# xingbpshen/nested-diffusion

Hardware: AMD Instinct MI355X
Metric: denoising-steps*images/sec (K=5,T=100,224^2) (higher is better)
Workload: dtype f32

## Files before the change

include/nested_diffusion.h:

```cpp
#ifndef NESTED_DIFFUSION_H
#define NESTED_DIFFUSION_H

#include <stddef.h>
#include <stdint.h>

#ifdef __cplusplus
extern "C" {
#endif

#define ND_OK 0
#define ND_ERR_ARG (-1)
#define ND_ERR_HIP (-2)
#define ND_ERR_STATE (-3)

#define ND_ACT_NONE 0
#define ND_ACT_SOFTPLUS 1
#define ND_ACT_RELU 2
#define ND_ACT_GELU 3

typedef struct nd_handle_s *nd_handle;

typedef struct {
    int32_t y_dim;
    int32_t data_dim;
// ... 21 lines not shown
    const float *lin2_w, *lin2_b, *emb2;
    const float *un2_w, *un2_b, *un2_mean, *un2_var;
    const float *lin3_w, *lin3_b, *emb3;
    const float *un3_w, *un3_b, *un3_mean, *un3_var;
    const float *lin4_w, *lin4_b;
} nd_member_weights;

const char *nd_last_error(void);
const char *nd_version(void);

int nd_create(const nd_config *cfg, nd_handle *out);
int nd_destroy(nd_handle h);
size_t nd_workspace_bytes(const nd_config *cfg);
int nd_bind_workspace(nd_handle h, void *workspace_dev, size_t bytes);

int nd_load_member(nd_handle h, int member, const nd_member_weights *w, void *stream);

int nd_set_schedule(nd_handle h, const float *alphas_dev, const float *omabs_dev, int T, void *stream);

int nd_encode(nd_handle h, int member0, int n_members, const float *x_dev, int B, void *stream);

int nd_eps_theta(nd_handle h, int member, const float *y_dev, const float *yhat_dev, int t,
                 float *eps_out_dev, int B, int mc, void *stream);

int nd_p_sample(nd_handle h, int member, const float *y_dev, const float *yhat_dev, const float *ymean_dev,
                const float *z_dev, int t, float *y_out_dev, int B, int mc, void *stream);

int nd_sample(nd_handle h, int member0, int n_members, const float *yhat_dev, const float *ymean_dev,
              const float *noise_dev, float *y0_out_dev, float *seq_out_dev, int B, int mc, int T,
              int use_graph, void *stream);

int nd_set_profiling(nd_handle h, int enable);
long long nd_resident_weight_bytes(nd_handle h, int block);
int nd_profile_read(nd_handle h, float *out_us, int *n_samples);
int nd_profile_probe_nodes(nd_handle h);

int nd_set_input_flag(nd_handle h, uint32_t *flag_host_visible);

int nd_set_loop_form(nd_handle h, int mode, float skew_us);
int nd_loop_form(nd_handle h);
int nd_persist_status(nd_handle h, int reset);

int nd_member_buffer(nd_handle h, int member, int which, float *dst_dev, int rows, void *stream);

size_t nd_packed_bytes(int R, int K, int dtype);
int nd_pack_rows(const float *src_dev, void *dst_packed_dev, int R, int K, int dtype, void *stream);

size_t nd_linear_workspace_bytes(int M, int K, int N, int dtype);
int nd_linear(const float *x_dev, const void *w_packed_dev, const float *scale_dev, const float *shift_dev,
              float *out_dev, int M, int K, int N, int act, int dtype, void *workspace_dev, size_t workspace_bytes,
              void *stream);

int nd_skinny_plan(int K, int N, int M, int n_members, int dtype, int mode, int *out6);
int nd_skinny_row_fragments(int M);

int nd_step_plan(int feature_dim, int M, int n_members, int dtype, int *out8);

size_t nd_gemm_workspace_bytes(int M, int K, int N, int dtype);
int nd_gemm_bias_act(const float *x_dev, const void *w_dev, const float *bias_dev, const float *residual_dev,
                     float *out_dev, int M, int K, int N, int act, int dtype, void *workspace_dev, size_t workspace_bytes,
                     void *stream);

size_t nd_split_bytes(int rows, int K);
int nd_split_rows(const float *x_dev, void *out_split_dev, int rows, int K, void *stream);
int nd_join_rows(const void *in_split_dev, float *x_dev, int rows, int K, void *stream);
size_t nd_gemm_split_workspace_bytes(int M, int K, int N);
// ... 168 lines not shown
```

nested_diffusion_amd/_lib.py:

```python
from __future__ import annotations

import ctypes as C
import os
from typing import Optional

HERE = os.path.dirname(os.path.abspath(__file__))
LIB_PATH = os.environ.get("ND_LIB_PATH") or os.path.join(HERE, "libnd_hip.so")

ND_ACT_NONE, ND_ACT_SOFTPLUS, ND_ACT_RELU, ND_ACT_GELU = 0, 1, 2, 3
ND_DTYPE_F32, ND_DTYPE_F16 = 0, 1
ND_DTYPE_F32_SPLIT = 2


def dtype_code(dtype) -> int:
    name = str(dtype).replace("torch.", "").lower()
    if name in ("f32", "fp32", "float32", "0"):
        return ND_DTYPE_F32
    if name in ("f16", "fp16", "float16", "half", "1"):
        return ND_DTYPE_F16
    raise ValueError(f"operand dtype must be 'f32' or 'f16', got {dtype!r}")

MEMBER_WEIGHT_FIELDS = [
    ("enc0_w", "encoder_x.0.weight"), ("enc0_b", "encoder_x.0.bias"),
    ("bn0_w", "encoder_x.1.weight"), ("bn0_b", "encoder_x.1.bias"),
    ("bn0_mean", "encoder_x.1.running_mean"), ("bn0_var", "encoder_x.1.running_var"),
    ("enc3_w", "encoder_x.3.weight"), ("enc3_b", "encoder_x.3.bias"),
    ("bn1_w", "encoder_x.4.weight"), ("bn1_b", "encoder_x.4.bias"),
    ("bn1_mean", "encoder_x.4.running_mean"), ("bn1_var", "encoder_x.4.running_var"),
    ("enc6_w", "encoder_x.6.weight"), ("enc6_b", "encoder_x.6.bias"),
    ("norm_w", "norm.weight"), ("norm_b", "norm.bias"),
    ("norm_mean", "norm.running_mean"), ("norm_var", "norm.running_var"),
    ("lin1_w", "lin1.lin.weight"), ("lin1_b", "lin1.lin.bias"), ("emb1", "lin1.embed.weight"),
    ("un1_w", "unetnorm1.weight"), ("un1_b", "unetnorm1.bias"),
    ("un1_mean", "unetnorm1.running_mean"), ("un1_var", "unetnorm1.running_var"),
    ("lin2_w", "lin2.lin.weight"), ("lin2_b", "lin2.lin.bias"), ("emb2", "lin2.embed.weight"),
    ("un2_w", "unetnorm2.weight"), ("un2_b", "unetnorm2.bias"),
    ("un2_mean", "unetnorm2.running_mean"), ("un2_var", "unetnorm2.running_var"),
    ("lin3_w", "lin3.lin.weight"), ("lin3_b", "lin3.lin.bias"), ("emb3", "lin3.embed.weight"),
    ("un3_w", "unetnorm3.weight"), ("un3_b", "unetnorm3.bias"),
    ("un3_mean", "unetnorm3.running_mean"), ("un3_var", "unetnorm3.running_var"),
    ("lin4_w", "lin4.weight"), ("lin4_b", "lin4.bias"),
]

# ... 30 lines not shown
    _fields_ = [("w_packed", C.c_void_p * 4), ("bias", C.c_void_p * 4)]


class NdAdamStep(C.Structure):
    _fields_ = [(n, C.c_float) for n in ("beta1", "one_minus_beta1", "beta2", "one_minus_beta2", "step_size", "sqrt_bc2", "eps")]


class NdBatchOut(C.Structure):
    _fields_ = [(n, C.c_void_p) for n in ("samples", "prob", "vote", "probs", "yhat")]


_vp, _i, _sz, _f = C.c_void_p, C.c_int, C.c_size_t, C.c_float
SIGNATURES = {
    "nd_last_error": (C.c_char_p, []),
    "nd_version": (C.c_char_p, []),
    "nd_create": (_i, [C.POINTER(NdConfig), C.POINTER(_vp)]),
    "nd_destroy": (_i, [_vp]),
    "nd_workspace_bytes": (_sz, [C.POINTER(NdConfig)]),
    "nd_bind_workspace": (_i, [_vp, _vp, _sz]),
    "nd_load_member": (_i, [_vp, _i, C.POINTER(NdMemberWeights), _vp]),
    "nd_set_schedule": (_i, [_vp, _vp, _vp, _i, _vp]),
    "nd_encode": (_i, [_vp, _i, _i, _vp, _i, _vp]),
    "nd_eps_theta": (_i, [_vp, _i, _vp, _vp, _i, _vp, _i, _i, _vp]),
    "nd_p_sample": (_i, [_vp, _i, _vp, _vp, _vp, _vp, _i, _vp, _i, _i, _vp]),
    "nd_sample": (_i, [_vp, _i, _i, _vp, _vp, _vp, _vp, _vp, _i, _i, _i, _i, _vp]),
    "nd_set_profiling": (_i, [_vp, _i]),
    "nd_set_input_flag": (_i, [_vp, _vp]),
    "nd_set_loop_form": (_i, [_vp, _i, C.c_float]),
    "nd_loop_form": (_i, [_vp]),
    "nd_persist_status": (_i, [_vp, _i]),
    "nd_profile_read": (_i, [_vp, C.POINTER(C.c_float), C.POINTER(_i)]),
    "nd_profile_probe_nodes": (_i, [_vp]),
    "nd_resident_weight_bytes": (C.c_longlong, [_vp, _i]),
    "nd_member_buffer": (_i, [_vp, _i, _i, _vp, _i, _vp]),
    "nd_seed": (_i, [_vp, C.c_uint64, C.c_uint32]),
    "nd_philox_normal": (_i, [_vp, _i, _i, _i, _i, _i, C.c_uint64, C.c_uint32, C.c_uint32, _vp]),
    "nd_philox_raw": (_i, [_vp, _vp, _i, C.c_uint32, C.c_uint32, _vp]),
    "nd_cond_workspace_bytes": (_sz, [C.POINTER(NdCondConfig)]),
    "nd_cond_create": (_i, [C.POINTER(NdCondConfig), C.POINTER(_vp)]),
    "nd_cond_destroy": (_i, [_vp]),
    "nd_cond_get_config": (C.POINTER(NdCondConfig), [_vp]),
    "nd_cond_bind_workspace": (_i, [_vp, _vp, _sz]),
    "nd_cond_set_patch_embed": (_i, [_vp, C.POINTER(NdPatchEmbedWeights)]),
    "nd_cond_set_block": (_i, [_vp, _i, C.POINTER(NdVitBlockWeights)]),
    "nd_cond_set_mlp": (_i, [_vp, _i, C.POINTER(NdMlpWeights)]),
    "nd_vit_block": (_i, [_vp, _i, _vp, _vp, _i, _i, _vp]),
    "nd_guiding_prediction": (_i, [_vp, _vp, _vp, _vp, _i, _vp]),
    "nd_predict_batch": (_i, [_vp, _vp, _vp, _vp, C.POINTER(NdBatchOut), _i, _i, _i, _f, _i, _vp]),
    "nd_packed_bytes": (_sz, [_i, _i, _i]),
    "nd_pack_rows": (_i, [_vp, _vp, _i, _i, _i, _vp]),
    "nd_linear_workspace_bytes": (_sz, [_i, _i, _i, _i]),
    "nd_linear": (_i, [_vp, _vp, _vp, _vp, _vp, _i, _i, _i, _i, _i, _vp, _sz, _vp]),
    "nd_skinny_plan": (_i, [_i, _i, _i, _i, _i, _i, C.POINTER(_i)]),
    "nd_step_plan": (_i, [_i, _i, _i, _i, C.POINTER(_i)]),
    "nd_skinny_row_fragments": (_i, [_i]),
    "nd_gemm_workspace_bytes": (_sz, [_i, _i, _i, _i]),
    "nd_gemm_bias_act": (_i, [_vp, _vp, _vp, _vp, _vp, _i, _i, _i, _i, _i, _vp, _sz, _vp]),
    "nd_split_bytes": (_sz, [_i, _i]),
    "nd_split_rows": (_i, [_vp, _vp, _i, _i, _vp]),
    "nd_join_rows": (_i, [_vp, _vp, _i, _i, _vp]),
    "nd_gemm_split_workspace_bytes": (_sz, [_i, _i, _i]),
    "nd_gemm_split": (_i, [_vp, _vp, _vp, _vp, _vp, _vp, _i, _i, _i, _i, _vp, _sz, _vp]),
    "nd_layernorm": (_i, [_vp, _vp, _vp, _vp, _i, _i, _f, _vp]),
    "nd_layernorm_split": (_i, [_vp, _vp, _vp, _vp, _i, _i, _f, _vp]),
    "nd_attention": (_i, [_vp, _vp, _i, _i, _i, _i, _i, _vp]),
    "nd_attention_split": (_i, [_vp, _vp, _i, _i, _i, _i, _vp]),
# ... 93 lines not shown
```

nested_diffusion_amd/csrc/nd_common.hpp:

```cpp
#pragma once
#include <type_traits>
#include <mutex>
#include <unordered_map>
#include <hip/hip_runtime.h>
#include <stdint.h>

typedef float f32x4 __attribute__((ext_vector_type(4)));
typedef _Float16 f16x8 __attribute__((ext_vector_type(8)));
typedef _Float16 f16x4 __attribute__((ext_vector_type(4)));

#define ND_ACT_NONE 0
#define ND_ACT_SOFTPLUS 1
#define ND_ACT_RELU 2
#define ND_ACT_GELU 3

__device__ __forceinline__ float nd_softplus(float x) {
#pragma clang fp contract(off)
    const float u = expf(-fabsf(x));
    const float w = 1.0f + u;
    const float c = (w - 1.0f) - u;
    const float r = fmaxf(x, 0.0f) + __builtin_fmaf(-c, __builtin_amdgcn_rcpf(w), logf(w));
    return x > 20.0f ? x : r;
}

// ... 140 lines not shown
}

typedef __attribute__((address_space(1))) const f32x4 nd_gf4;
template <bool NT>
__device__ __forceinline__ float4 nd_ld16(const float* p) {
    const nd_gf4* g = (const nd_gf4*)p;
    const f32x4 v = NT ? __builtin_nontemporal_load(g) : *g;
    return make_float4(v[0], v[1], v[2], v[3]);
}

#ifdef ND_WG_TIMING
__device__ long long* nd_dbg_times = nullptr;
#endif

__device__ __forceinline__ float nd_ldg(const float* p) {
    return *(const __attribute__((address_space(1))) float*)p;
}

#ifndef ND_PF_TWO
#define ND_PF_TWO 0
#endif
#ifndef ND_PF_LEAD
#define ND_PF_LEAD 0
#endif
struct SkinnyDesc {
    const float* x;
    const float* w;
    const float* scale;
    const float* shift;
    float* out;
    const float* pw;
    float* part;
    int K, N, C, act, out_packed;
    int keep;
    const float* pf;
};

#define ND_INLINE_DESCS 8
struct SkinnyInline { SkinnyDesc d[ND_INLINE_DESCS]; };

template <typename T>
__device__ __forceinline__ T nd_ldc(const __attribute__((address_space(4))) void* p) {
    static_assert(sizeof(T) % 4 == 0, "word-sized structs only");
    T out;
    const __attribute__((address_space(4))) uint32_t* w = (const __attribute__((address_space(4))) uint32_t*)p;
    uint32_t* o = reinterpret_cast<uint32_t*>(&out);
#pragma unroll
    for (unsigned i = 0; i < sizeof(T) / 4; ++i) o[i] = w[i];
    return out;
}

#define ND_SKINNY_STATIC_LDS (60 * 1024)
__host__ __device__ constexpr int nd_skinny_red_bytes(int waves, int nf, int mt) { return waves * nf * mt * 1024; }
template <int MT, int NF, int WAVES, int U, int MODE, bool NT, int H = 0>
__global__ __launch_bounds__(WAVES * 64) void k_skinny(SkinnyInline di, const SkinnyDesc* __restrict__ table, int nm,
                                                       int M, int t, int cps) {
    const int tid = threadIdx.x, lane = tid & 63;
#ifdef ND_WG_TIMING
    const long long dbg_t0 = wall_clock64();
#endif
    const int wave = __builtin_amdgcn_readfirstlane(tid >> 6);
    typedef const __attribute__((address_space(4))) char* nd_cbytes;
    const nd_cbytes dsrc = table ? (nd_cbytes)(uintptr_t)table : (nd_cbytes)__builtin_amdgcn_kernarg_segment_ptr();
    const int K = nd_ldc<SkinnyDesc>(dsrc).K, N = nd_ldc<SkinnyDesc>(dsrc).N;
    const int nch = H ? K >> 5 : K >> 4, nfr = (N + 15) >> 4, mtiles = (M + 15) >> 4;
    const int wpm = gridDim.x / nm;
    const int g = blockIdx.x / wpm, j = blockIdx.x - g * wpm;
    const int base = nfr / wpm, rem = nfr - base * wpm;
    const int nact = base + (j < rem ? 1 : 0);
// ... 80 lines not shown
                                const float wv = jj == 0 ? w[u][f].x : jj == 1 ? w[u][f].y : jj == 2 ? w[u][f].z : w[u][f].w;
                                const float xv = jj == 0 ? x[u][mt].x : jj == 1 ? x[u][mt].y : jj == 2 ? x[u][mt].z : x[u][mt].w;
                                acc[f][mt] = __builtin_amdgcn_mfma_f32_16x16x4f32(wv, xv, acc[f][mt], 0, 0, 0);
                            }
                        }
        };
        auto G = [&](int i) { return min(wave + i * WAVES, glast); };
        int i = 0;
        if (ngw > 0) LD(wA, xA, G(0));
        constexpr int NL = U * (NFA + MT), NM = U * (H ? 1 : 4) * NFA * MT, MR = NM / NL > 0 ? NM / NL : 1;
#define ND_MIX()                                                                                     \
        _Pragma("unroll") for (int q_ = 0; q_ < NL; ++q_) {                                          \
            __builtin_amdgcn_sched_group_barrier(0x020, 1, 0);                                       \
            __builtin_amdgcn_sched_group_barrier(0x008, MR, 0);                                      \
        }                                                                                            \
        __builtin_amdgcn_sched_barrier(0);
        const int pf_at = ngw > ND_PF_LEAD ? (ngw - ND_PF_LEAD) & ~1 : 0;
        for (; i + 1 < ngw; i += 2) {
            if (MODE != 2 && pfp[0] && i == pf_at && ND_PF_LEAD > 0) {
                pfv += nd_ldg(pfp[0]) + nd_ldg(pfp[1]);
                if (ND_PF_TWO) pfv += nd_ldg(pfp[0] + (size_t)WAVES * U * 256) + nd_ldg(pfp[1] + (size_t)WAVES * U * 256);
            }
            LD(wB, xB, G(i + 1));
            MMA(wA, xA);
            ND_MIX()
            LD(wA, xA, G(i + 2));
            MMA(wB, xB);
            ND_MIX()
        }
#undef ND_MIX
        if (ND_PF_LEAD == 0 && MODE != 2 && pfp[0]) pfv += nd_ldg(pfp[0]) + nd_ldg(pfp[1]);
        if (i < ngw) MMA(wA, xA);
    };
    const bool nt_here = NT && !d.keep;
    if (nact == NF) {
        if (nt_here) run(std::true_type{}, std::true_type{});
        else run(std::false_type{}, std::true_type{});
    } else {
        if (nt_here) run(std::true_type{}, std::false_type{});
        else run(std::false_type{}, std::false_type{});
    }
    for (int c = ngroups * U + wave; c < nck; c += WAVES) {
#pragma unroll
        for (int f = 0; f < NF; ++f) {
            const float4 w4 = nd_ld16<false>(wp[f] + (size_t)c * 256 + lane4);
            const float wv[4] = {w4.x, w4.y, w4.z, w4.w};
#pragma unroll
            for (int mt = 0; mt < MT; ++mt) {
                const float4 x4 = nd_ld16<false>(xp[mt] + (size_t)c * 256 + lane4);
                const float xv[4] = {x4.x, x4.y, x4.z, x4.w};
                if (H) acc[f][mt] = __builtin_amdgcn_mfma_f32_16x16x32_f16(nd_as_h8(w4), nd_as_h8(x4), acc[f][mt], 0, 0, 0);
                else {
#pragma unroll
                    for (int jj = 0; jj < 4; ++jj) acc[f][mt] = __builtin_amdgcn_mfma_f32_16x16x4f32(wv[jj], xv[jj], acc[f][mt], 0, 0, 0);
                }
            }
        }
    }
#ifdef ND_WG_TIMING
    const long long dbg_t1 = wall_clock64();
#endif
    if (ND_PF_LEAD < 0 && MODE != 2 && pfp[0]) {
        pfv += nd_ldg(pfp[0]) + nd_ldg(pfp[1]);
        if (ND_PF_TWO) pfv += nd_ldg(pfp[0] + (size_t)WAVES * U * 256) + nd_ldg(pfp[1] + (size_t)WAVES * U * 256);
    }
    if (MODE != 2) {
        if (tid < NF * 16) { ssc[tid >> 4][tid & 15] = r_sc; ssh[tid >> 4][tid & 15] = r_sh; }
// ... 337 lines not shown
```

nested_diffusion_amd/csrc/nd_persist.hip:

```cpp
#include "nd_persist.hpp"
#include <cstddef>

typedef unsigned u32x4 __attribute__((ext_vector_type(4)));
typedef __attribute__((address_space(1))) unsigned* nd_gu32;

#ifdef ND_PERSIST_TIMING
__device__ long long* nd_persist_times = nullptr;
extern "C" int nd_debug_set_persist_times(void* dev_ptr) {
    return hipMemcpyToSymbol(HIP_SYMBOL(nd_persist_times), &dev_ptr, sizeof(void*)) == hipSuccess ? 0 : -1;
}
#define PS_STAMP(k) do { const long long now_ = wall_clock64(); ps_acc[k] += now_ - ps_last; ps_last = now_; } while (0)
#else
#define PS_STAMP(k) do { } while (0)
#endif

#define PS_WAVES 4
#define PS_MT 2
#define PS_U 2

__device__ __forceinline__ unsigned ps_ld_sc1(const unsigned* p) { return __hip_atomic_load((nd_gu32)p, __ATOMIC_RELAXED, __HIP_MEMORY_SCOPE_AGENT); }
__device__ __forceinline__ void ps_st_sc1(unsigned* p, unsigned v) { __hip_atomic_store((nd_gu32)p, v, __ATOMIC_RELAXED, __HIP_MEMORY_SCOPE_AGENT); }
__device__ __forceinline__ float ps_ldf_sc1(const float* p) {
    return __hip_atomic_load((__attribute__((address_space(1))) float*)p, __ATOMIC_RELAXED, __HIP_MEMORY_SCOPE_AGENT);
}
// ... 93 lines not shown
#ifdef ND_PERSIST_TIMING
    long long ps_acc[9] = {0, 0, 0, 0, 0, 0, 0, 0, 0}, ps_last = 0;
#endif

    {
        const SkinnyDesc d3 = PS_ARG_G(ka, SkinnyDesc, l3, g);
        const StepIO io = PS_ARG(ka, StepIO, io);
        for (int e = tid; e < NF * C * 16; e += WAVES * 64) {
            const int f = e / (C * 16), c = (e / 16) % C, nl = e & 15;
            const int n = min(fi0 + f, nfr - 1) * 16 + nl;
            smem[L::pws + e] = (f < nact) ? nd_ldg(d3.pw + (size_t)c * F + n) : 0.f;
        }
        for (int p = tid; p < pairs; p += WAVES * 64) {
            const int m = p / C, c = p - m * C, b = m % B;
            smem[L::syh + p] = nd_ldg(io.yhat + g * io.yhat_ms + (size_t)b * C + c);
            smem[L::sym + p] = nd_ldg(io.ymean + g * io.ymean_ms + (size_t)b * C + c);
        }
    }
    __syncthreads();

    const int ngroups = nch / U;
    const int ngw = ngroups > wave ? (ngroups - wave + WAVES - 1) / WAVES : 0;
    const int glast = ngroups > 0 ? ngroups - 1 : 0;
    float (*const red)[NF * MT * 256] = reinterpret_cast<float (*)[NF * MT * 256]>(smem + L::red);

    auto poison = [&]() {
        if (j != 0) return;
        const StepIO io = PS_ARG(ka, StepIO, io);
        for (int p = tid; p < pairs; p += WAVES * 64) ND_GW(io.y0_out)[g * io.y0_ms + p] = __builtin_nanf("");
    };

    auto layer = [&](auto modec, int t) -> bool {
        constexpr int MODE = decltype(modec)::value;
        const float* wbase; const float* xbase; float* obase; int keep;
        float r_sc = 1.0f, r_sh = 0.0f;
        {
            const SkinnyDesc d = MODE == 0 ? PS_ARG_G(ka, SkinnyDesc, l2, g) : PS_ARG_G(ka, SkinnyDesc, l3, g);
            wbase = d.w; xbase = d.x; obase = MODE == 0 ? d.out : d.part; keep = d.keep;
            if (tid < NF * 16) {
                const int n = min(min(fi0 + (tid >> 4), nfr - 1) * 16 + (tid & 15), F - 1);
                r_sc = nd_ldg(d.scale + (size_t)t * F + n);
                r_sh = nd_ldg(d.shift + (size_t)t * F + n);
            }
        }
        const __amdgpu_buffer_rsrc_t rx = ps_rsrc(xbase);
        const float* wp[NF];
#pragma unroll
        for (int f = 0; f < NF; ++f) wp[f] = wbase + (size_t)min(fi0 + f, nfr - 1) * nch * 256;
        f32x4 acc[NF][MT];
#pragma unroll
        for (int f = 0; f < NF; ++f)
#pragma unroll
            for (int mt = 0; mt < MT; ++mt) acc[f][mt] = f32x4{0.f, 0.f, 0.f, 0.f};
        bool alive = true;
        auto run = [&](auto ntc, auto fullc) {
            constexpr bool NTV = decltype(ntc)::value, FULL = decltype(fullc)::value;
            constexpr int NFA = FULL ? NF : (NF > 1 ? NF - 1 : 1);
            float4 wA[U][NFA], xA[U][MT], wB[U][NFA], xB[U][MT];
            auto LDW = [&](float4 (&w)[U][NFA], int grp) {
                const size_t go = (size_t)grp * U * 256;
#pragma unroll
                for (int u = 0; u < U; ++u)
#pragma unroll
                    for (int f = 0; f < NFA; ++f) w[u][f] = nd_ld16<NTV>(wp[f] + go + u * 256 + lane4);
            };
            auto LDX = [&](float4 (&x)[U][MT], int grp) {
#pragma unroll
                for (int u = 0; u < U; ++u)
#pragma unroll
                    for (int mt = 0; mt < MT; ++mt)
                        x[u][mt] = ps_ld16_sc1(rx, lane * 16, ((min(mt, mtiles - 1) * nch + grp * U + u) * 1024));
// ... 300 lines not shown
```

nested_diffusion_amd/csrc/nd_sampler.hip:

```cpp
#include "nd_common.hpp"
#include "nd_step.hpp"
#include "nd_cond_gemm.hpp"
#include "nd_b9.hpp"
#include "nd_persist.hpp"
#include "nd_rng.hpp"
#include "../../include/nested_diffusion.h"

#include <map>
#include <string>
#include <tuple>
#include <vector>
#include <cstdio>
#include <cstdarg>
#include <cstring>
#include <cstdlib>

static thread_local std::string g_err;
extern "C" const char* nd_last_error(void) { return g_err.c_str(); }
#ifdef ND_WG_TIMING
int nd_debug_set_wg_times_m0(void*); int nd_debug_set_wg_times_m1(void*); int nd_debug_set_wg_times_m2(void*);
extern "C" int nd_debug_set_wg_times(void* dev_ptr) {
    return (nd_debug_set_wg_times_m0(dev_ptr) | nd_debug_set_wg_times_m1(dev_ptr) | nd_debug_set_wg_times_m2(dev_ptr)) ? -1 : 0;
}
#endif
// ... 289 lines not shown
        case 1: return (void*)k_step_final<1>;
        case 2: return (void*)k_step_final<2>;
        case 3: return (void*)k_step_final<3>;
        case 4: return (void*)k_step_final<4>;
        case 5: return (void*)k_step_final<5>;
        case 6: return (void*)k_step_final<6>;
        case 7: return (void*)k_step_final<7>;
        default: return (void*)k_step_final<8>;
    }
}

__global__ void k_fold_bn(float* scale, float* shift, const float* lin_b, const float* bn_w, const float* bn_b,
                          const float* bn_mean, const float* bn_var, int N) {
    const int n = blockIdx.x * blockDim.x + threadIdx.x;
    if (n >= N) return;
    const double s = (double)bn_w[n] / sqrt((double)bn_var[n] + 1e-5);
    const double o = (double)bn_b[n] - (double)bn_mean[n] * s;
    scale[n] = (float)s;
    shift[n] = (float)(s * (double)lin_b[n] + o);
}
__global__ void k_fold_steps(float* A, float* Cc, const float* emb, const float* lin_b, const float* bn_w, const float* bn_b,
                             const float* bn_mean, const float* bn_var, int T, int N) {
    const size_t i = (size_t)blockIdx.x * blockDim.x + threadIdx.x;
    if (i >= (size_t)T * N) return;
    const int n = (int)(i % N);
    const double s = (double)bn_w[n] / sqrt((double)bn_var[n] + 1e-5);
    const double o = (double)bn_b[n] - (double)bn_mean[n] * s;
    const double g = (double)emb[i];
    A[i] = (float)(s * g);
    Cc[i] = (float)(s * g * (double)lin_b[n] + o);
}

#define ND_KEEP_BYTES 208.0e6
enum { L_ENC0 = 0, L_ENC1 = 1, L_ENC2 = 2, L_LIN2 = 3, L_LIN3 = 4, L_LIN2S = 5, L_LIN3S = 6, L_COUNT = 7 };

struct MemberHost {
    bool loaded = false;
    float *sc0, *sh0, *sc1, *sh1, *sc2, *sh2;
    float *A[3], *Cc[3];
    float *w_enc0, *w_enc3, *w_enc6, *w_lin2, *w_lin3;
    float *w_lin1, *w_lin4, *b_lin4;
    float *e0, *e1, *xe, *ybuf, *h1, *h2, *epart, *splitk;
    void *w_lin2s = nullptr, *w_lin3s = nullptr, *h1s = nullptr, *h2s = nullptr;
    bool h_split = false;
};

struct GraphKey {
    int m0, nm, B, mc, T;
    const void *yhat, *ymean, *noise, *y0, *seq;
    bool operator<(const GraphKey& o) const {
        return std::tie(m0, nm, B, mc, T, yhat, ymean, noise, y0, seq) <
               std::tie(o.m0, o.nm, o.B, o.mc, o.T, o.yhat, o.ymean, o.noise, o.y0, o.seq);
    }
};

int nd_guiding_prediction_first(nd_cond c, const float* images, float* logits_out, float* yhat_out, int B, int n_used, void* stream);
unsigned long long nd_cond_serial(nd_cond c);

struct BatchKey {
    unsigned long long cond;
    const void *images, *noise, *samples, *prob, *vote, *probs, *yhat;
    int B, mc, T;
    unsigned temp_bits;
    bool profiling;
    bool operator<(const BatchKey& o) const {
        return std::tie(cond, images, noise, samples, prob, vote, probs, yhat, B, mc, T, temp_bits, profiling) <
               std::tie(o.cond, o.images, o.noise, o.samples, o.prob, o.vote, o.probs, o.yhat, o.B, o.mc, o.T, o.temp_bits, o.profiling);
    }
};

struct nd_handle_s {
    nd_config cfg{};
    char* ws = nullptr;
    size_t ws_bytes = 0;
    std::vector<MemberHost> members;
    MemberDev* members_dev = nullptr;
    SkinnyDesc* descs_dev = nullptr;
    std::vector<SkinnyDesc> descs_host;
    std::vector<MemberDev> members_host;
    SkinnyDesc* spk_dev = nullptr;
    SplitKEpiDesc* spke_dev = nullptr;
    float *alphas = nullptr, *omabs = nullptr;
    float* xpack = nullptr;
    float* tile_ws = nullptr;
    bool b9 = false;
    unsigned long long* rng_state = nullptr;
    unsigned* input_seq = nullptr;
    unsigned* input_flag = nullptr;
    unsigned* persist_bar = nullptr;
    int persist_mode = 0;
    int persist_skew_ticks = 0;
    bool persist_last = false;
    float* noise_ws = nullptr;
    float* logits_ws = nullptr;
    int sched_T = 0;
    int NT = 0, S0 = 0;
    bool enc_splitk = false;
    int half = 0;
    std::map<GraphKey, hipGraphExec_t> graphs;
    std::map<BatchKey, hipGraphExec_t> batch_graphs;
    hipStream_t capture_stream = nullptr;
    int encoded_B = -1;
    bool profiling = false;
    std::vector<hipEvent_t> probe_events;
    int probe_steps = 0;
    int probe_nodes = 0;
};

static inline size_t al256(size_t x) { return (x + 255) & ~(size_t)255; }

struct Carver {
    char* base; size_t off = 0;
    template <typename T> T* take(size_t count) {
        T* p = base ? reinterpret_cast<T*>(base + off) : nullptr;
        off = al256(off + count * sizeof(T));
        return p;
    }
};

static void carve(nd_handle_s* h, char* base, size_t* total) {
    const nd_config& c = h->cfg;
    const size_t K = c.n_members, H = c.hidden_dim, F = c.feature_dim, T = c.n_steps, C = c.y_dim, D = c.data_dim;
    const size_t mB = c.max_batch, mM = c.max_rows;
    const size_t pB = ((mB + 15) / 16) * 16, pM = ((mM + 15) / 16) * 16;
    h->NT = (int)((F + 15) / 16);
    h->half = c.operand_dtype == ND_DTYPE_F16;
    const size_t wdiv = h->half ? 2 : 1;
    h->enc_splitk = nd_use_splitk(c.data_dim);
    h->S0 = h->enc_splitk ? nd_skinny_launch<2>(c.data_dim, c.hidden_dim, c.max_batch, 1, h->half).S : 0;
    Carver cv{base};
    h->members_dev = cv.take<MemberDev>(K);
// ... 103 lines not shown
    HIP_CHECK(hipMemset(h->rng_state, 0, 2 * sizeof(unsigned long long)));
    HIP_CHECK(hipMemset(h->persist_bar, 0, ND_PERSIST_BAR_WORDS * sizeof(unsigned)));
    HIP_CHECK(hipMemset(h->input_seq, 0, sizeof(unsigned)));
    return ND_OK;
}

extern "C" int nd_seed(nd_handle h, uint64_t seed, uint32_t first_image) {
    if (!h || !h->ws) return nd_set_err(ND_ERR_STATE, "workspace not bound");
    const unsigned long long st[2] = {(unsigned long long)seed, (unsigned long long)first_image << 32};
    HIP_CHECK(hipDeviceSynchronize());
    HIP_CHECK(hipMemcpy(h->rng_state, st, sizeof st, hipMemcpyHostToDevice));
    return ND_OK;
}

extern "C" int nd_set_schedule(nd_handle h, const float* alphas_dev, const float* omabs_dev, int T, void* stream) {
    if (!h || !h->ws) return nd_set_err(ND_ERR_STATE, "workspace not bound");
    if (!alphas_dev || !omabs_dev) return nd_set_err(ND_ERR_ARG, "NULL schedule");
    if (T < 1 || T > h->cfg.n_steps) return nd_set_err(ND_ERR_ARG, "T=%d outside [1,%d]", T, h->cfg.n_steps);
    hipStream_t st = (hipStream_t)stream;
    HIP_CHECK(hipMemcpyAsync(h->alphas, alphas_dev, sizeof(float) * T, hipMemcpyDeviceToDevice, st));
    HIP_CHECK(hipMemcpyAsync(h->omabs, omabs_dev, sizeof(float) * T, hipMemcpyDeviceToDevice, st));
    h->sched_T = T;
    return ND_OK;
}

static void launch_pack(const float* src, float* dst, int R, int K, int half, hipStream_t st) {
    const size_t n4 = (size_t)((R + 15) / 16) * 16 * K / (half ? 8 : 4);
    const size_t want = (n4 + 255) / 256;
    const dim3 grid((unsigned)(want > 8192 ? 8192 : want));
    if (half) hipLaunchKernelGGL(k_pack_rows_h, grid, dim3(256), 0, st, src, reinterpret_cast<_Float16*>(dst), R, K);
    else hipLaunchKernelGGL(k_pack_rows, grid, dim3(256), 0, st, src, dst, R, K);
}

extern "C" int nd_load_member(nd_handle h, int k, const nd_member_weights* w, void* stream) {
    if (!h || !h->ws) return nd_set_err(ND_ERR_STATE, "workspace not bound");
    if (k < 0 || k >= h->cfg.n_members) return nd_set_err(ND_ERR_ARG, "member %d out of range", k);
    if (!w) return nd_set_err(ND_ERR_ARG, "weights is NULL");
    const void* const* pp = reinterpret_cast<const void* const*>(w);
    for (size_t i = 0; i < sizeof(nd_member_weights) / sizeof(void*); ++i)
        if (!pp[i]) return nd_set_err(ND_ERR_ARG, "nd_member_weights pointer #%zu is NULL", i);
    hipStream_t st = (hipStream_t)stream;
    const nd_config& c = h->cfg;
    const int H = c.hidden_dim, F = c.feature_dim, T = c.n_steps, C = c.y_dim, D = c.data_dim;
    MemberHost& m = h->members[k];
    auto g1 = [](int n) { return dim3((n + 255) / 256); };
    hipLaunchKernelGGL(k_fold_bn, g1(H), dim3(256), 0, st, m.sc0, m.sh0, w->enc0_b, w->bn0_w, w->bn0_b, w->bn0_mean, w->bn0_var, H);
    hipLaunchKernelGGL(k_fold_bn, g1(H), dim3(256), 0, st, m.sc1, m.sh1, w->enc3_b, w->bn1_w, w->bn1_b, w->bn1_mean, w->bn1_var, H);
    hipLaunchKernelGGL(k_fold_bn, g1(F), dim3(256), 0, st, m.sc2, m.sh2, w->enc6_b, w->norm_w, w->norm_b, w->norm_mean, w->norm_var, F);
    const float* embs[3] = {w->emb1, w->emb2, w->emb3};
    const float* lb[3] = {w->lin1_b, w->lin2_b, w->lin3_b};
    const float* bw[3] = {w->un1_w, w->un2_w, w->un3_w};
    const float* bb[3] = {w->un1_b, w->un2_b, w->un3_b};
    const float* bm[3] = {w->un1_mean, w->un2_mean, w->un3_mean};
    const float* bv[3] = {w->un1_var, w->un2_var, w->un3_var};
    const size_t tot = (size_t)T * F;
    for (int l = 0; l < 3; ++l)
        hipLaunchKernelGGL(k_fold_steps, dim3((unsigned)((tot + 255) / 256)), dim3(256), 0, st, m.A[l], m.Cc[l], embs[l], lb[l],
                           bw[l], bb[l], bm[l], bv[l], T, F);
    launch_pack(w->enc0_w, m.w_enc0, H, D, h->half, st);
    launch_pack(w->enc3_w, m.w_enc3, H, H, h->half, st);
    launch_pack(w->enc6_w, m.w_enc6, F, H, h->half, st);
    launch_pack(w->lin2_w, m.w_lin2, F, F, h->half, st);
    launch_pack(w->lin3_w, m.w_lin3, F, F, h->half, st);
    if (h->b9) {
        int rc = nd_split_rows(w->lin2_w, m.w_lin2s, F, F, st);
        if (rc == ND_OK) rc = nd_split_rows(w->lin3_w, m.w_lin3s, F, F, st);
        if (rc != ND_OK) return rc;
        HIP_CHECK(nd_cond_gemm_b9_prepare());
    }
    HIP_CHECK(hipMemcpyAsync(m.w_lin1, w->lin1_w, sizeof(float) * F * 2 * C, hipMemcpyDeviceToDevice, st));
    HIP_CHECK(hipMemcpyAsync(m.w_lin4, w->lin4_w, sizeof(float) * C * F, hipMemcpyDeviceToDevice, st));
    HIP_CHECK(hipMemcpyAsync(m.b_lin4, w->lin4_b, sizeof(float) * C, hipMemcpyDeviceToDevice, st));
    HIP_CHECK(hipGetLastError());

    MemberDev md{m.w_lin1, m.b_lin4, m.A[0], m.Cc[0], m.xe, m.h1, m.ybuf, m.epart, h->half};
    const int opk = h->half ? 2 : 1;
    SkinnyDesc ds[L_COUNT];
    ds[L_ENC0] = SkinnyDesc{h->xpack, m.w_enc0, m.sc0, m.sh0, m.e0, nullptr, nullptr, D, H, C, ND_ACT_SOFTPLUS, opk};
    ds[L_ENC1] = SkinnyDesc{m.e0, m.w_enc3, m.sc1, m.sh1, m.e1, nullptr, nullptr, H, H, C, ND_ACT_SOFTPLUS, opk};
    ds[L_ENC2] = SkinnyDesc{m.e1, m.w_enc6, m.sc2, m.sh2, m.xe, nullptr, nullptr, H, F, C, ND_ACT_NONE, 1};
    ds[L_LIN2] = SkinnyDesc{m.h1, m.w_lin2, m.A[1], m.Cc[1], m.h2, nullptr, nullptr, F, F, C, ND_ACT_SOFTPLUS, opk};
    ds[L_LIN3] = SkinnyDesc{m.h2, m.w_lin3, m.A[2], m.Cc[2], nullptr, m.w_lin4, m.epart, F, F, C, ND_ACT_SOFTPLUS, 0};
    if (!getenv("ND_NO_XPREFETCH")) { ds[L_LIN2].pf = m.w_lin3; ds[L_LIN3].pf = m.w_lin2; }
    ds[L_LIN2S] = ds[L_LIN2]; ds[L_LIN3S] = ds[L_LIN3];
    if (h->b9) {
        ds[L_LIN2S].x = (const float*)m.h1s; ds[L_LIN2S].w = (const float*)m.w_lin2s; ds[L_LIN2S].out = (float*)m.h2s; ds[L_LIN2S].out_packed = 3;
        ds[L_LIN3S].x = (const float*)m.h2s; ds[L_LIN3S].w = (const float*)m.w_lin3s;
    }
    {
        const double mat = (double)F * F * (h->half ? 2.0 : 4.0);
        const char* keep_mb = getenv("ND_KEEP_MB");
        const int n_keep = (int)((keep_mb ? atof(keep_mb) * 1e6 : ND_KEEP_BYTES) / mat);
        ds[L_LIN2].keep = k < n_keep;
        ds[L_LIN3].keep = c.n_members + k < n_keep;
        if (const char* plan = getenv("ND_KEEP_PLAN")) {
            int a = 0, b = 0;
            if (sscanf(plan, "%d,%d", &a, &b) == 2) { ds[L_LIN2].keep = k < a; ds[L_LIN3].keep = k < b; }
        }
    }
    HIP_CHECK(hipStreamSynchronize(st));
    HIP_CHECK(hipMemcpy(h->members_dev + k, &md, sizeof md, hipMemcpyHostToDevice));
    h->members_host.resize(c.n_members);
    h->descs_host.resize((size_t)L_COUNT * c.n_members);
    h->members_host[k] = md;
    for (int l = 0; l < L_COUNT; ++l) {
        h->descs_host[(size_t)l * c.n_members + k] = ds[l];
        HIP_CHECK(hipMemcpy(h->descs_dev + (size_t)l * c.n_members + k, &ds[l], sizeof(SkinnyDesc), hipMemcpyHostToDevice));
    }
    if (h->enc_splitk) {
        SkinnyDesc sd{h->xpack, m.w_enc0, nullptr, nullptr, nullptr, nullptr, m.splitk, D, H, C, ND_ACT_NONE, 0};
        SplitKEpiDesc se{m.splitk, m.sc0, m.sh0, m.e0, H, 0 , ND_ACT_SOFTPLUS, opk};
        HIP_CHECK(hipMemcpy(h->spk_dev + k, &sd, sizeof sd, hipMemcpyHostToDevice));
        HIP_CHECK(hipMemcpy(h->spke_dev + k, &se, sizeof se, hipMemcpyHostToDevice));
    }
    m.loaded = true;
    drop_graphs(h);
    return ND_OK;
}

static int check_range(nd_handle_s* h, int m0, int nm) {
    if (!h || !h->ws) return nd_set_err(ND_ERR_STATE, "workspace not bound");
    if (m0 < 0 || nm < 1 || m0 + nm > h->cfg.n_members) return nd_set_err(ND_ERR_ARG, "member range [%d,%d) invalid", m0, m0 + nm);
    for (int k = m0; k < m0 + nm; ++k)
        if (!h->members[k].loaded) return nd_set_err(ND_ERR_STATE, "member %d not loaded", k);
    return ND_OK;
}

template <int MODE>
static hipError_t launch_skinny(const SkinnyDesc* table, int K, int N, int M, int t, int nm, int half, hipStream_t st) {
    return nd_launch_skinny(nd_skinny_launch<MODE>(K, N, M, nm, half), SkinnyDesc{}, table, nm, M, t, st);
}
// ... 56 lines not shown
    HIP_CHECK(launch_skinny<0>(h->descs_dev + (size_t)L_ENC1 * K + m0, H, H, B, 0, nm, h->half, st));
    HIP_CHECK(launch_skinny<0>(h->descs_dev + (size_t)L_ENC2 * K + m0, H, F, B, 0, nm, h->half, st));
    HIP_CHECK(hipGetLastError());
    h->encoded_B = B;
    return ND_OK;
}

extern "C" int nd_member_buffer(nd_handle h, int k, int which, float* dst_dev, int rows, void* stream) {
    if (!h || !dst_dev) return nd_set_err(ND_ERR_ARG, "bad argument");
    if (k < 0 || k >= h->cfg.n_members) return nd_set_err(ND_ERR_ARG, "member out of range");
    if (which < 0 || which > 4) return nd_set_err(ND_ERR_ARG, "which=%d unknown", which);
    if (rows < 1 || rows > h->cfg.max_rows) return nd_set_err(ND_ERR_ARG, "rows out of range");
    const bool enc = which == 0 || which >= 3;
    if (enc && rows > h->cfg.max_batch) return nd_set_err(ND_ERR_ARG, "%s holds at most max_batch rows", which == 0 ? "xe" : which == 3 ? "e0" : "e1");
    if (!h->ws) return nd_set_err(ND_ERR_STATE, "workspace not bound");
    MemberHost& m = h->members[k];
    const float* src = which == 0 ? m.xe : which == 1 ? m.h1 : which == 2 ? m.h2 : which == 3 ? m.e0 : m.e1;
    const int W = which >= 3 ? h->cfg.hidden_dim : h->cfg.feature_dim;
    if (!enc && m.h_split) return nd_join_rows(which == 1 ? m.h1s : m.h2s, dst_dev, rows, W, stream);
    const size_t n4 = (size_t)((rows + 15) / 16) * 16 * W / 4;
    if (h->half && which != 0)
        hipLaunchKernelGGL(k_unpack_rows_h, dim3((unsigned)((n4 / 2 + 255) / 256)), dim3(256), 0, (hipStream_t)stream,
                           reinterpret_cast<const _Float16*>(src), dst_dev, rows, W);
    else
        hipLaunchKernelGGL(k_unpack_rows, dim3((unsigned)((n4 + 255) / 256)), dim3(256), 0, (hipStream_t)stream, src, dst_dev, rows, W);
    HIP_CHECK(hipGetLastError());
    return ND_OK;
}

extern "C" long long nd_resident_weight_bytes(nd_handle h, int block) {
    if (!h || block < 0 || block > 1 || h->descs_host.empty()) return -1;
    const int K = h->cfg.n_members, F = h->cfg.feature_dim;
    long long n = 0;
    for (int k = 0; k < K; ++k)
        if (h->members[k].loaded && h->descs_host[(size_t)(block ? L_LIN3 : L_LIN2) * K + k].keep) n += (long long)F * F * (h->half ? 2 : 4);
    return n;
}

extern "C" int nd_set_profiling(nd_handle h, int enable) {
    if (!h) return nd_set_err(ND_ERR_ARG, "handle is NULL");
    if (h->profiling != (enable != 0)) drop_graphs(h);
    h->profiling = enable != 0;
    return ND_OK;
}

extern "C" int nd_set_loop_form(nd_handle h, int mode, float skew_us) {
    if (!h) return nd_set_err(ND_ERR_ARG, "handle is NULL");
    if (mode != 0 && mode != 1) return nd_set_err(ND_ERR_ARG, "mode must be 0 (per-step kernels) or 1 (one launch per loop)");
    if (skew_us > 1e6f) return nd_set_err(ND_ERR_ARG, "skew_us out of range");
    h->persist_mode = mode;
    if (skew_us >= 0.f) h->persist_skew_ticks = (int)(skew_us * 100.0f);
    drop_graphs(h);
    return ND_OK;
}

extern "C" int nd_loop_form(nd_handle h) { return h && h->persist_last ? 1 : 0; }

extern "C" int nd_persist_status(nd_handle h, int reset) {
    if (!h || !h->ws) return nd_set_err(ND_ERR_STATE, "workspace not bound");
    HIP_CHECK(hipDeviceSynchronize());
    unsigned flag = 0;
    HIP_CHECK(hipMemcpy(&flag, h->persist_bar + ND_PERSIST_ERR_WORD, sizeof flag, hipMemcpyDeviceToHost));
    if (reset && flag) HIP_CHECK(hipMemset(h->persist_bar, 0, ND_PERSIST_BAR_WORDS * sizeof(unsigned)));
    return flag ? 1 : 0;
}

static int count_event_record_nodes(hipGraph_t g) {
    size_t n = 0;
    if (hipGraphGetNodes(g, nullptr, &n) != hipSuccess) return -1;
// ... 407 lines not shown
```

nested_diffusion_amd/engine.py:

```python
from __future__ import annotations

import ctypes as C
import os
from typing import Dict, Optional, Sequence, Tuple

import torch

from . import _lib
from ._lib import MEMBER_WEIGHT_FIELDS, NdBatchOut, NdConfig, NdMemberWeights, check, ptr


def _require_gpu(device) -> torch.device:
    device = torch.device(device)
    if device.type != "cuda" or not torch.cuda.is_available():
        raise _lib.NdError("nested_diffusion_amd needs an MI355X (torch device 'cuda'); there is no CPU fallback")
    return device


class EnsembleEngine:

    def __init__(self, y_dim: int, data_dim: int, hidden_dim: int, feature_dim: int, n_steps: int,
                 n_members: int = 1, max_batch: int = 32, max_rows: Optional[int] = None, device="cuda", dtype="f32"):
        self.device = _require_gpu(device)
        self.lib = _lib.load()
# ... 101 lines not shown
        check(self.lib.nd_set_loop_form(self.h, 1 if one_launch else 0, float(skew_us)), "nd_set_loop_form")

    def loop_form(self) -> str:
        return "one_launch" if self.lib.nd_loop_form(self.h) else "graph_nodes"

    def persist_status(self, reset: bool = False) -> bool:
        rc = self.lib.nd_persist_status(self.h, 1 if reset else 0)
        if rc < 0:
            check(rc, "nd_persist_status")
        if rc != 0:
            raise _lib.NdError("one-launch sampling loop: a barrier wait was abandoned (the grid was not resident at once -- another "
                               "process on this device?); results of that call are invalid.  ND_PERSIST=0 selects the per-step form")
        return True

    def set_profiling(self, enable: bool) -> None:
        check(self.lib.nd_set_profiling(self.h, 1 if enable else 0), "nd_set_profiling")

    def profile_read(self):
        torch.cuda.current_stream(self.device).synchronize()
        us = (C.c_float * 4)()
        n = C.c_int(0)
        check(self.lib.nd_profile_read(self.h, us, C.byref(n)), "nd_profile_read")
        self.probe_overhead_us = float(us[3])
        return float(us[0]), float(us[1]), float(us[3]), int(n.value)

    def probe_nodes(self) -> int:
        return int(self.lib.nd_profile_probe_nodes(self.h))

    def resident_weight_bytes(self) -> Tuple[int, int]:
        a, b = self.lib.nd_resident_weight_bytes(self.h, 0), self.lib.nd_resident_weight_bytes(self.h, 1)
        if a < 0 or b < 0:
            raise _lib.NdError("nd_resident_weight_bytes: members not loaded")
        return int(a), int(b)

    def step_plan(self, M: int, n_members: Optional[int] = None) -> Dict[str, object]:
        out = (C.c_int * 8)()
        n_members = self.K if n_members is None else n_members
        check(self.lib.nd_step_plan(self.F, int(M), int(n_members), self.dtype, out), "nd_step_plan")
        tile = bool(out[0])
        b9 = tile and self.dtype == _lib.ND_DTYPE_F32 and self.F % 32 == 0 and n_members <= 8 and not os.environ.get("ND_STEP_F32_MFMA")
        name = (("k_cond_gemm_b9<{0,1}> (LDS-tiled 128x128 ConditionalLinear blocks on the bf16 matrix pipe, nine exact bf16 pair products "
                 "per fp32 product, K members per launch)" if b9 else
                 "k_cond_gemm<{0,1}> (LDS-tiled 128x128 f32-MFMA ConditionalLinear blocks, K members per launch)") if tile else
                "k_skinny<MT,NF,4,U,{0,1}> (weight-streaming lin2 / lin3+lin4 ConditionalLinear blocks, K members per launch)")
        plan = {"kernel": "k_cond_gemm" if tile else "k_skinny", "b9": bool(b9), "name": name, "workgroups": out[1], "whole_tiles": out[2],
                "remainder_tiles": out[3], "split": out[4], "partials": out[5], "TM": out[6], "TN": out[7]}
        if not tile:
            o6 = (C.c_int * 6)()
            check(self.lib.nd_skinny_plan(self.F, self.F, int(M), int(n_members), self.dtype, 1, o6), "nd_skinny_plan")
            mt = self.lib.nd_skinny_row_fragments(int(M))
            if mt < 1:
                check(mt, "nd_skinny_row_fragments")
            plan["stream"] = {"grid": (o6[0], o6[1], o6[2]), "NF": o6[3], "MT": mt, "chunks_per_slab": o6[4], "threads": o6[5]}
        return plan

    def static_buffers(self, n_members: int, B: int, mc: int, T: int, seq: bool) -> Dict[str, torch.Tensor]:
        key = (n_members, B, mc, T, seq)
        buf = self._static.get(key)
        if buf is None:
            M, C_ = B * mc, self.C
            dev = self.device
            buf = {"yhat": torch.empty(n_members, B, C_, device=dev), "ymean": torch.empty(n_members, B, C_, device=dev),
                   "noise": torch.empty(n_members, T, M, C_, device=dev), "y0": torch.empty(n_members, M, C_, device=dev)}
            if seq:
                buf["seq"] = torch.empty(n_members, T + 1, M, C_, device=dev)
            self._static[key] = buf
# ... 84 lines not shown
```

Baseline: 790,500.

## Make cache residency of skinny-layer weights a per-fragment range plan

Replaces the per-member boolean 'keep' flag (which decided whether a whole FxF weight matrix is loaded with temporal hints or non-temporal loads) with a per-workgroup fragment range [keep_lo, keep_hi). A planner fills these ranges under a byte budget using several layouts: whole matrices, matrices plus a fractional one, or a heavy-first slice spread evenly across members. New API calls let the residency be set at runtime. The f32 default keeps the matrix layout with the same budget, so f32 behaviour should be close to the old whole-matrix policy. f16 defaults to a heavy+even layout with a slightly smaller budget. The kernel now checks the range per workgroup, which adds a small amount of per-workgroup logic.

```diff
diff --git a/include/nested_diffusion.h b/include/nested_diffusion.h
--- a/include/nested_diffusion.h
+++ b/include/nested_diffusion.h
@@ -77,6 +77,13 @@
 
 int nd_set_profiling(nd_handle h, int enable);
 long long nd_resident_weight_bytes(nd_handle h, int block);
+#define ND_RESIDENCY_MATRIX 0
+#define ND_RESIDENCY_MATRIX_FRAC 1
+#define ND_RESIDENCY_HEAVY 2
+#define ND_RESIDENCY_HEAVY_EVEN 3
+int nd_residency_plan(int n_members, int feature_dim, int dtype, long long budget_bytes, int layout, unsigned short *out);
+int nd_set_residency(nd_handle h, int layout, long long budget_bytes);
+int nd_set_residency_ranges(nd_handle h, const unsigned short *ranges);
 int nd_profile_read(nd_handle h, float *out_us, int *n_samples);
 int nd_profile_probe_nodes(nd_handle h);
 
diff --git a/nested_diffusion_amd/_lib.py b/nested_diffusion_amd/_lib.py
--- a/nested_diffusion_amd/_lib.py
+++ b/nested_diffusion_amd/_lib.py
@@ -9,6 +9,7 @@
 
 ND_ACT_NONE, ND_ACT_SOFTPLUS, ND_ACT_RELU, ND_ACT_GELU = 0, 1, 2, 3
 ND_DTYPE_F32, ND_DTYPE_F16 = 0, 1
+RESIDENCY_LAYOUTS = {"matrix": 0, "matrix+frac": 1, "heavy": 2, "heavy+even": 3}
 ND_DTYPE_F32_SPLIT = 2
 
 
@@ -105,6 +106,9 @@
     "nd_profile_read": (_i, [_vp, C.POINTER(C.c_float), C.POINTER(_i)]),
     "nd_profile_probe_nodes": (_i, [_vp]),
     "nd_resident_weight_bytes": (C.c_longlong, [_vp, _i]),
+    "nd_residency_plan": (_i, [_i, _i, _i, C.c_longlong, _i, C.POINTER(C.c_ushort)]),
+    "nd_set_residency": (_i, [_vp, _i, C.c_longlong]),
+    "nd_set_residency_ranges": (_i, [_vp, C.POINTER(C.c_ushort)]),
     "nd_member_buffer": (_i, [_vp, _i, _i, _vp, _i, _vp]),
     "nd_seed": (_i, [_vp, C.c_uint64, C.c_uint32]),
     "nd_philox_normal": (_i, [_vp, _i, _i, _i, _i, _i, C.c_uint64, C.c_uint32, C.c_uint32, _vp]),
diff --git a/nested_diffusion_amd/csrc/nd_common.hpp b/nested_diffusion_amd/csrc/nd_common.hpp
--- a/nested_diffusion_amd/csrc/nd_common.hpp
+++ b/nested_diffusion_amd/csrc/nd_common.hpp
@@ -196,9 +196,13 @@
     const float* pw;
     float* part;
     int K, N, C, act, out_packed;
-    int keep;
+    uint16_t keep_lo, keep_hi;
     const float* pf;
 };
+static_assert(sizeof(SkinnyDesc) == 88 && offsetof(SkinnyDesc, pf) == 80, "SkinnyDesc travels by value in the kernel arguments: its layout is fixed");
+__host__ __device__ __forceinline__ bool nd_wg_kept(const SkinnyDesc& d, int fi0, int nact) {
+    return fi0 >= (int)d.keep_lo && fi0 + nact <= (int)d.keep_hi;
+}
 
 #define ND_INLINE_DESCS 8
 struct SkinnyInline { SkinnyDesc d[ND_INLINE_DESCS]; };
@@ -345,7 +349,7 @@
         if (ND_PF_LEAD == 0 && MODE != 2 && pfp[0]) pfv += nd_ldg(pfp[0]) + nd_ldg(pfp[1]);
         if (i < ngw) MMA(wA, xA);
     };
-    const bool nt_here = NT && !d.keep;
+    const bool nt_here = NT && !nd_wg_kept(d, fi0, nact);
     if (nact == NF) {
         if (nt_here) run(std::true_type{}, std::true_type{});
         else run(std::false_type{}, std::true_type{});
diff --git a/nested_diffusion_amd/csrc/nd_persist.hip b/nested_diffusion_amd/csrc/nd_persist.hip
--- a/nested_diffusion_amd/csrc/nd_persist.hip
+++ b/nested_diffusion_amd/csrc/nd_persist.hip
@@ -149,11 +149,11 @@
 
     auto layer = [&](auto modec, int t) -> bool {
         constexpr int MODE = decltype(modec)::value;
-        const float* wbase; const float* xbase; float* obase; int keep;
+        const float* wbase; const float* xbase; float* obase; bool keep;
         float r_sc = 1.0f, r_sh = 0.0f;
         {
             const SkinnyDesc d = MODE == 0 ? PS_ARG_G(ka, SkinnyDesc, l2, g) : PS_ARG_G(ka, SkinnyDesc, l3, g);
-            wbase = d.w; xbase = d.x; obase = MODE == 0 ? d.out : d.part; keep = d.keep;
+            wbase = d.w; xbase = d.x; obase = MODE == 0 ? d.out : d.part; keep = nd_wg_kept(d, fi0, nact);
             if (tid < NF * 16) {
                 const int n = min(min(fi0 + (tid >> 4), nfr - 1) * 16 + (tid & 15), F - 1);
                 r_sc = nd_ldg(d.scale + (size_t)t * F + n);
diff --git a/nested_diffusion_amd/csrc/nd_sampler.hip b/nested_diffusion_amd/csrc/nd_sampler.hip
--- a/nested_diffusion_amd/csrc/nd_sampler.hip
+++ b/nested_diffusion_amd/csrc/nd_sampler.hip
@@ -345,6 +345,55 @@
 }
 
 #define ND_KEEP_BYTES 208.0e6
+#define ND_KEEP_LAYOUT ND_RESIDENCY_MATRIX
+#define ND_KEEP_BYTES_H 201.0e6
+#define ND_KEEP_LAYOUT_H ND_RESIDENCY_HEAVY_EVEN
+#define ND_RES_CUS 256
+
+static void nd_residency_fill(int K, int F, int half, long long budget, int layout, uint16_t* out) {
+    const int nfr = (F + 15) / 16;
+    const long long fb = 16LL * F * (half ? 2 : 4);
+    for (int i = 0; i < 4 * K; ++i) out[i] = 0;
+    long long left = budget > 0 ? budget : 0;
+    auto hi = [&](int layer, int k) -> uint16_t& { return out[((size_t)layer * K + k) * 2 + 1]; };
+    if (layout == ND_RESIDENCY_HEAVY || layout == ND_RESIDENCY_HEAVY_EVEN) {
+        const int wpm = ND_RES_CUS / K > 0 ? ND_RES_CUS / K : 1;
+        const int nh = std::min(nfr, (nfr + wpm - 1) / wpm);
+        for (int layer = 0; layer < 2; ++layer)
+            for (int k = 0; k < K; ++k) {
+                if (left < nh * fb) return;
+                hi(layer, k) = (uint16_t)nh;
+                left -= nh * fb;
+            }
+    }
+    if (layout == ND_RESIDENCY_HEAVY_EVEN) {
+        for (int layer = 0; layer < 2; ++layer) {
+            const int room = nfr - hi(layer, 0);
+            const int share = (int)std::min<long long>(room, left / (K * fb));
+            for (int k = 0; k < K; ++k) hi(layer, k) = (uint16_t)(hi(layer, k) + share);
+            left -= (long long)share * K * fb;
+            if (share < room) return;
+        }
+        return;
+    }
+    for (int layer = 0; layer < 2; ++layer)
+        for (int k = 0; k < K; ++k) {
+            const long long cost = (long long)(nfr - hi(layer, k)) * fb;
+            if (left >= cost) { hi(layer, k) = (uint16_t)nfr; left -= cost; continue; }
+            if (layout != ND_RESIDENCY_MATRIX) hi(layer, k) = (uint16_t)(hi(layer, k) + left / fb);
+            return;
+        }
+}
+
+extern "C" int nd_residency_plan(int n_members, int feature_dim, int dtype, long long budget_bytes, int layout, unsigned short* out) {
+    if (!out) return nd_set_err(ND_ERR_ARG, "out is NULL");
+    const int half = dtype == ND_DTYPE_F16, mul = half ? 32 : 16;
+    if ((dtype != ND_DTYPE_F32 && dtype != ND_DTYPE_F16) || n_members < 1 || n_members > 255 || feature_dim < mul || (feature_dim % mul) ||
+        feature_dim / 16 > 65535 || budget_bytes < 0 || layout < ND_RESIDENCY_MATRIX || layout > ND_RESIDENCY_HEAVY_EVEN)
+        return nd_set_err(ND_ERR_ARG, "bad shape / dtype / budget / layout");
+    nd_residency_fill(n_members, feature_dim, half, budget_bytes, layout, out);
+    return ND_OK;
+}
 enum { L_ENC0 = 0, L_ENC1 = 1, L_ENC2 = 2, L_LIN2 = 3, L_LIN3 = 4, L_LIN2S = 5, L_LIN3S = 6, L_COUNT = 7 };
 
 struct MemberHost {
@@ -410,6 +459,10 @@
     int NT = 0, S0 = 0;
     bool enc_splitk = false;
     int half = 0;
+    int res_layout = -1;
+    long long res_budget = -1;
+    std::vector<uint16_t> res_ranges;
+    bool res_set = false;
     std::map<GraphKey, hipGraphExec_t> graphs;
     std::map<BatchKey, hipGraphExec_t> batch_graphs;
     hipStream_t capture_stream = nullptr;
@@ -579,6 +632,36 @@
     else hipLaunchKernelGGL(k_pack_rows, grid, dim3(256), 0, st, src, dst, R, K);
 }
 
+static void residency_ranges(const nd_handle_s* h, std::vector<uint16_t>& r) {
+    const int K = h->cfg.n_members, F = h->cfg.feature_dim;
+    if (h->res_set && !h->res_ranges.empty()) { r = h->res_ranges; return; }
+    r.assign((size_t)4 * K, 0);
+    long long budget = h->res_budget;
+    int layout = h->res_layout;
+    if (!h->res_set) {
+        budget = (long long)(h->half ? ND_KEEP_BYTES_H : ND_KEEP_BYTES);
+        layout = h->half ? ND_KEEP_LAYOUT_H : ND_KEEP_LAYOUT;
+        if (const char* keep_mb = getenv("ND_KEEP_MB")) {
+            budget = (long long)(atof(keep_mb) * 1e6);
+            layout = ND_RESIDENCY_MATRIX;
+        }
+    }
+    nd_residency_fill(K, F, h->half, budget, layout, r.data());
+    if (const char* plan = h->res_set ? nullptr : getenv("ND_KEEP_PLAN")) {
+        int a = 0, b = 0;
+        if (sscanf(plan, "%d,%d", &a, &b) == 2)
+            for (int k = 0; k < K; ++k) {
+                r[(size_t)k * 2] = 0; r[(size_t)k * 2 + 1] = (uint16_t)(k < a ? (F + 15) / 16 : 0);
+                r[((size_t)K + k) * 2] = 0; r[((size_t)K + k) * 2 + 1] = (uint16_t)(k < b ? (F + 15) / 16 : 0);
+            }
+    }
+}
+
+static void residency_apply(const std::vector<uint16_t>& r, int K, int k, SkinnyDesc& lin2, SkinnyDesc& lin3) {
+    lin2.keep_lo = r[(size_t)k * 2]; lin2.keep_hi = r[(size_t)k * 2 + 1];
+    lin3.keep_lo = r[((size_t)K + k) * 2]; lin3.keep_hi = r[((size_t)K + k) * 2 + 1];
+}
+
 extern "C" int nd_load_member(nd_handle h, int k, const nd_member_weights* w, void* stream) {
     if (!h || !h->ws) return nd_set_err(ND_ERR_STATE, "workspace not bound");
     if (k < 0 || k >= h->cfg.n_members) return nd_set_err(ND_ERR_ARG, "member %d out of range", k);
@@ -635,15 +718,9 @@
         ds[L_LIN3S].x = (const float*)m.h2s; ds[L_LIN3S].w = (const float*)m.w_lin3s;
     }
     {
-        const double mat = (double)F * F * (h->half ? 2.0 : 4.0);
-        const char* keep_mb = getenv("ND_KEEP_MB");
-        const int n_keep = (int)((keep_mb ? atof(keep_mb) * 1e6 : ND_KEEP_BYTES) / mat);
-        ds[L_LIN2].keep = k < n_keep;
-        ds[L_LIN3].keep = c.n_members + k < n_keep;
-        if (const char* plan = getenv("ND_KEEP_PLAN")) {
-            int a = 0, b = 0;
-            if (sscanf(plan, "%d,%d", &a, &b) == 2) { ds[L_LIN2].keep = k < a; ds[L_LIN3].keep = k < b; }
-        }
+        std::vector<uint16_t> r;
+        residency_ranges(h, r);
+        residency_apply(r, c.n_members, k, ds[L_LIN2], ds[L_LIN3]);
     }
     HIP_CHECK(hipStreamSynchronize(st));
     HIP_CHECK(hipMemcpy(h->members_dev + k, &md, sizeof md, hipMemcpyHostToDevice));
@@ -766,9 +843,47 @@
     if (!h || block < 0 || block > 1 || h->descs_host.empty()) return -1;
     const int K = h->cfg.n_members, F = h->cfg.feature_dim;
     long long n = 0;
-    for (int k = 0; k < K; ++k)
-        if (h->members[k].loaded && h->descs_host[(size_t)(block ? L_LIN3 : L_LIN2) * K + k].keep) n += (long long)F * F * (h->half ? 2 : 4);
+    for (int k = 0; k < K; ++k) {
+        const SkinnyDesc& d = h->descs_host[(size_t)(block ? L_LIN3 : L_LIN2) * K + k];
+        if (h->members[k].loaded && d.keep_hi > d.keep_lo) n += (long long)(d.keep_hi - d.keep_lo) * 16 * F * (h->half ? 2 : 4);
+    }
     return n;
+}
+
+static int residency_commit(nd_handle_s* h) {
+    drop_graphs(h);
+    if (h->descs_host.empty()) return ND_OK;
+    const int K = h->cfg.n_members;
+    std::vector<uint16_t> r;
+    residency_ranges(h, r);
+    HIP_CHECK(hipDeviceSynchronize());
+    for (int k = 0; k < K; ++k) {
+        if (!h->members[k].loaded) continue;
+        SkinnyDesc* d2 = &h->descs_host[(size_t)L_LIN2 * K + k];
+        SkinnyDesc* d3 = &h->descs_host[(size_t)L_LIN3 * K + k];
+        residency_apply(r, K, k, *d2, *d3);
+        HIP_CHECK(hipMemcpy(h->descs_dev + (size_t)L_LIN2 * K + k, d2, sizeof(SkinnyDesc), hipMemcpyHostToDevice));
+        HIP_CHECK(hipMemcpy(h->descs_dev + (size_t)L_LIN3 * K + k, d3, sizeof(SkinnyDesc), hipMemcpyHostToDevice));
+    }
+    return ND_OK;
+}
+
+extern "C" int nd_set_residency(nd_handle h, int layout, long long budget_bytes) {
+    if (!h) return nd_set_err(ND_ERR_ARG, "handle is NULL");
+    if (layout < ND_RESIDENCY_MATRIX || layout > ND_RESIDENCY_HEAVY_EVEN) return nd_set_err(ND_ERR_ARG, "layout=%d unknown", layout);
+    if (budget_bytes < 0) return nd_set_err(ND_ERR_ARG, "budget_bytes must be >= 0");
+    h->res_layout = layout; h->res_budget = budget_bytes; h->res_ranges.clear(); h->res_set = true;
+    return residency_commit(h);
+}
+
+extern "C" int nd_set_residency_ranges(nd_handle h, const unsigned short* ranges) {
+    if (!h || !ranges) return nd_set_err(ND_ERR_ARG, "handle / ranges is NULL");
+    const int K = h->cfg.n_members, nfr = (h->cfg.feature_dim + 15) / 16;
+    for (int i = 0; i < 2 * K; ++i)
+        if (ranges[2 * i] > ranges[2 * i + 1] || ranges[2 * i + 1] > nfr)
+            return nd_set_err(ND_ERR_ARG, "range %d: [%d, %d) not inside [0, %d]", i, ranges[2 * i], ranges[2 * i + 1], nfr);
+    h->res_ranges.assign(ranges, ranges + (size_t)4 * K); h->res_set = true;
+    return residency_commit(h);
 }
 
 extern "C" int nd_set_profiling(nd_handle h, int enable) {
diff --git a/nested_diffusion_amd/engine.py b/nested_diffusion_amd/engine.py
--- a/nested_diffusion_amd/engine.py
+++ b/nested_diffusion_amd/engine.py
@@ -157,6 +157,15 @@
         if a < 0 or b < 0:
             raise _lib.NdError("nd_resident_weight_bytes: members not loaded")
         return int(a), int(b)
+
+    def set_residency(self, layout: str, budget_bytes: int) -> None:
+        check(self.lib.nd_set_residency(self.h, _lib.RESIDENCY_LAYOUTS[layout], int(budget_bytes)), "nd_set_residency")
+
+    def set_residency_ranges(self, ranges) -> None:
+        flat = [int(v) for layer in ranges for pair in layer for v in pair]
+        if len(flat) != 4 * self.K:
+            raise ValueError(f"ranges must be [2][{self.K}][2]")
+        check(self.lib.nd_set_residency_ranges(self.h, (C.c_ushort * len(flat))(*flat)), "nd_set_residency_ranges")
 
     def step_plan(self, M: int, n_members: Optional[int] = None) -> Dict[str, object]:
         out = (C.c_int * 8)()
```

Result: no change. 788,000 (-0.3%).
